# norlab-ulaval/mask_bev

Hardware: AMD Instinct MI355X
Metric: LiDAR scans/sec fwd+bwd, 120k-pt 512x512 BEV 100q (higher is better)
Workload: dtype bf16; 1 GPU; semantic_kitti_512: 120000 pts/scan, 512x512 BEV, 100 queries; scans_per_gpu=4, global_batch=4, parallelism=dp1, step=fwd + Hungarian loss + bwd + AdamW; inputs device-resident, launch=hip-graph, tuned_gemm_table=True, k3_adam_fused=True

## Files before the change

include/maskbev_hip.h:

```cpp
#ifndef MASKBEV_HIP_H_
#define MASKBEV_HIP_H_

#include <stddef.h>
#include <stdint.h>

#ifdef __cplusplus
extern "C" {
#endif

typedef enum {
  MBV_OK = 0,
  MBV_ERR_BAD_ARG = -1,
  MBV_ERR_WORKSPACE = -2,
  MBV_ERR_UNSUPPORTED = -3
} mbv_status;

int mbv_abi_version(void);

#define MBV_DT_F32 0
#define MBV_DT_BF16 1
#define MBV_DT_F16 2

size_t mbv_voxelize_workspace_bytes(int64_t total_points, int32_t batch, int64_t cells_per_scan);

// ... 377 lines not shown
int mbv_groupnorm_fwd(const void* x, int32_t x_dtype, int64_t batch, int32_t channels, int32_t h, int32_t w,
                      int32_t groups, const float* gamma, const float* beta, float eps, const void* add,
                      int32_t add_dtype, int32_t add_h, int32_t add_w, int32_t relu, void* y, int32_t y_dtype, float* mean,
                      float* rstd, void* workspace, size_t workspace_bytes, void* stream);
int mbv_groupnorm_bwd(const void* dy, int32_t dy_dtype, const void* x, int32_t x_dtype, const float* mean,
                      const float* rstd, const float* gamma, const float* beta, int64_t batch, int32_t channels, int32_t h,
                      int32_t w, int32_t groups, int32_t relu, void* dx, int32_t dx_dtype, float* dgamma, float* dbeta,
                      int32_t accumulate, float* plane_sums, void* stream);

size_t mbv_gemm16_tn_group_workspace_bytes(const int64_t* m, const int64_t* n, const int64_t* k, int32_t count);

int mbv_gemm16_tn_group(const void* const* g, const void* const* x, float* const* dw, const int64_t* m, const int64_t* n,
                        const int64_t* k, const int64_t* ldg, const int64_t* ldx, int32_t count, int32_t dtype,
                        void* workspace, size_t workspace_bytes, void* stream);

#define MBV_RC_LOAD 0
#define MBV_RC_STORE 1
#define MBV_RC_GEMM 2
#define MBV_RC_LN 3
#define MBV_RC_LN_BWD 4
#define MBV_RC_ADD 5
#define MBV_RC_COLSUM 6
#define MBV_RC_FFN 7
#define MBV_RC_FFN_IO 8
#define MBV_RC_SUM 9
#define MBV_RC_ACCUM 4
#define MBV_RC_RELU 8
#define MBV_RC_MASK 16
#define MBV_RC_SAVE_SUM 32
#define MBV_RC_SLICE 64
#define MBV_RC_SPLIT 64
#define MBV_RC_FRAG 128
#define MBV_RC_OWNER(j) (((j) + 1) << 8)
#define MBV_TR_MAX 96
typedef struct MbvRowStage {
  int32_t op;
  int16_t dst, src, src2, reserved;
  int32_t n, k, flags, ld, ld2;
  const void* p0;
  const void* p1;
  const void* p2;
} MbvRowStage;
int mbv_rowchain_max_stages(void);
int mbv_rowchain_slots(void);
int mbv_rowchain_run(const MbvRowStage* stages, int32_t num_stages, int32_t rows, int32_t q_mod, float eps,
                     int32_t wdtype, void* stream);
int mbv_rowchain_run_split(const MbvRowStage* stages, int32_t num_stages, int32_t rows, int32_t q_mod, float eps,
                           int32_t wdtype, int32_t split, void* stream);
int mbv_fragment_group(const void* const* src, void* const* dst, const int32_t* rows, const int32_t* cols,
                       const int32_t* ld, const int32_t* transposed, int32_t n, void* stream);
int mbv_copy_group(const void* const* src, void* const* dst, const int64_t* bytes, int32_t n, void* stream);
int mbv_transpose_group(const void* const* src, void* const* dst, const int32_t* rows, const int32_t* cols, int32_t n,
                        int32_t elem_size, void* stream);

int mbv_gemm32s_supported(int32_t layout, int64_t m, int64_t n, int64_t k);

int mbv_f32_absmax_group(const float* const* x, const int64_t* rows, const int64_t* cols, const int64_t* ld,
                         uint32_t* const* out, int32_t count, void* stream);

int mbv_ln_bound_group(const float* const* gamma, const float* const* beta, const int32_t* c, uint32_t* const* records,
                       int32_t count, void* stream);

int mbv_gemm32s_nt(const float* x, const float* w, const float* bias, float* out, float* out_pre, int64_t m, int64_t n,
                   int64_t k, int64_t ldx, int64_t ldw, int64_t ldo, const uint32_t* amax_x, const uint32_t* amax_w,
                   uint32_t* amax_out, int32_t act, int32_t batch, int64_t stride_x, int64_t stride_w, int64_t stride_o,
                   void* stream);

int mbv_gemm32s_nn(const float* g, const float* w, float* out, int64_t m, int64_t n, int64_t k, int64_t ldg, int64_t ldw,
                   int64_t ldo, const uint32_t* amax_g, const uint32_t* amax_w, uint32_t* amax_out, int32_t batch,
                   int64_t stride_g, int64_t stride_w, int64_t stride_o, void* stream);

size_t mbv_gemm32s_tn_workspace_bytes(int64_t m, int64_t n, int64_t k);
int mbv_gemm32s_tn_acc(const float* g, const float* x, float* dw, int64_t m, int64_t n, int64_t k, int64_t ldg, int64_t ldx,
                       const uint32_t* amax_g, const uint32_t* amax_x, void* workspace, size_t workspace_bytes,
                       void* stream);

int mbv_patch_embed32_supported(int64_t batch, int64_t channels, int64_t h, int64_t w, int64_t embed);
int mbv_patch_embed32_fwd(const float* image, const float* weight, const float* bias, float* out, int64_t batch,
                          int64_t channels, int64_t h, int64_t w, int64_t embed, const uint32_t* amax_image,
                          const uint32_t* amax_w, void* stream);
int mbv_patch_embed32_bwd_image(const float* d_out, const float* weight, float* d_image, int64_t batch, int64_t channels,
                                int64_t h, int64_t w, int64_t embed, const uint32_t* amax_g, const uint32_t* amax_w,
                                void* stream);
size_t mbv_patch_embed32_bwd_weight_workspace_bytes(int64_t batch, int64_t channels, int64_t h, int64_t w, int64_t embed);
int mbv_patch_embed32_bwd_weight(const float* d_out, const float* image, float* d_weight, int64_t batch, int64_t channels,
                                 int64_t h, int64_t w, int64_t embed, const uint32_t* amax_g, const uint32_t* amax_image,
                                 void* workspace, size_t workspace_bytes, void* stream);


size_t mbv_gemm32s_tn_group_workspace_bytes(const int64_t* m, const int64_t* n, const int64_t* k, int32_t count);
int mbv_gemm32s_tn_group(const float* const* g, const float* const* x, float* const* dw, const int64_t* m, const int64_t* n,
                         const int64_t* k, const int64_t* ldg, const int64_t* ldx, const uint32_t* const* amax_g,
                         const uint32_t* const* amax_x, int32_t count, void* workspace, size_t workspace_bytes, void* stream);

int64_t mbv_conv_rows(int64_t batch, int64_t H, int64_t W);
int mbv_conv_pad_rows(const void* src, void* dst, int64_t batch, int64_t C, int64_t H, int64_t W, int32_t elem_size, void* stream);
int mbv_conv_unpad_rows(const void* src, void* dst, int64_t batch, int64_t C, int64_t H, int64_t W, int32_t elem_size,
                        void* stream);
int mbv_conv3x3_gemm32s(const float* rows, const float* wm, float* out_rows, int64_t batch, int64_t H, int64_t W, int64_t C,
                        int64_t cout, const uint32_t* amax_rows, const uint32_t* amax_w, uint32_t* amax_out, void* stream);
int mbv_conv3x3_gemm16(const void* rows, const void* wm, void* out_rows, int64_t batch, int64_t H, int64_t W, int64_t C,
                       int64_t cout, int32_t dtype, int32_t out_f32, void* stream);

int64_t mbv_gemm32s_nn_part_rows(int64_t m, int32_t batch);
int mbv_gemm32s_nn_act(const float* g, const float* w, float* out, const float* pre, float* parts, size_t parts_bytes,
                       int64_t m, int64_t n, int64_t k, int64_t ldg, int64_t ldw, int64_t ldo, int64_t ldpre,
// ... 25 lines not shown
```

mask_bev_amd/_lib.py:

```python
from __future__ import annotations

import ctypes
import os
from ctypes import c_double, c_float, c_int32, c_int64, c_size_t, c_void_p
from typing import Dict, List, Tuple

_PKG_DIR = os.path.dirname(os.path.abspath(__file__))
LIB_PATH = os.path.join(_PKG_DIR, 'libmaskbev_hip.so')

ABI_VERSION = 59


class MaskBevHipError(RuntimeError):
    pass


_P = c_void_p
_F = c_float
_I = c_int32
_L = c_int64
_D = c_double

SIGNATURES: Dict[str, Tuple[object, List[object]]] = {
    'mbv_abi_version': (ctypes.c_int, []),
    'mbv_voxelize_workspace_bytes': (c_size_t, [_L, _I, _L]),
    'mbv_voxelize': (ctypes.c_int, [_P, _I, _L, _P, _I, _F, _F, _F, _F, _F, _F, _F, _F, _F, _I, _I, _I, _I, _I, _I, _L,
                                    _P, _P, _P, _P, _P, _P, _P, c_size_t, _P]),
    'mbv_gather_voxels': (ctypes.c_int, [_P, _I, _P, _L, _I, _P, _P]),
    'mbv_pfn_decorate': (ctypes.c_int, [_P, _I, _P, _P, _P, _P, _L, _I, _F, _F, _F, _F, _F, _F, _P, _P, _P]),
    'mbv_pfn_stats': (ctypes.c_int, [_P, _P, _P, _P, _P, _L, _I, _I, _P, _P]),
    'mbv_pfn_bn_finalize': (ctypes.c_int, [_P, c_double, _P, _P, _F, _F, _I, _P, _P, _I, _P, _P, _P, _P, _P]),
    'mbv_pfn_apply_max': (ctypes.c_int, [_P, _P, _P, _P, _P, _P, _L, _I, _I, _P, _P, _P, _P]),
    'mbv_pfn_bwd_route': (ctypes.c_int, [_P, _P, _P, _P, _P, _P, _P, _I, _P, _P, _P, _P, _L, _I, _I, _P, _P, _P]),
    'mbv_pfn_bwd_bn': (ctypes.c_int, [_P, _P, _P, _P, _P, _P, _P, _P, c_double, _I, _P, _P, _L, _I, _I, _P, _P]),
    'mbv_scatter_layernorm_workspace_bytes': (c_size_t, [_I]),
    'mbv_scatter_layernorm_patch_supported': (ctypes.c_int, [_I, _I, _I, _I]),
    'mbv_scatter_layernorm_fwd': (ctypes.c_int, [_P, _P, _P, _P, _P, _I, _I, _I, _I, _F, _I, _I, _P, _P, _P, c_size_t,
                                                 _P, _P, _P]),
    'mbv_scatter_layernorm_fwd2': (ctypes.c_int, [_P, _P, _P, _P, _P, _I, _I, _I, _I, _F, _I, _I, _P, _P, _P, c_size_t,
                                                  _P, _P, _P, _P]),
    'mbv_scatter_layernorm_bwd': (ctypes.c_int, [_P, _I, _I, _P, _P, _P, _P, _P, _I, _I, _I, _I, _L, _P, _P, _P, _I, _P,
                                                 c_size_t, _P, _P, _P]),
    'mbv_scatter_layernorm_bwd_adamw': (ctypes.c_int, [_P, _I, _I, _P, _P, _P, _P, _P, _P, _I, _I, _I, _I, _L, _P, _P, _P, _P, _P,
                                                       _P, _P, _I, _F, _F, _F, _F, _F, _L, _I, _P, c_size_t, _P, _P, _P]),
    'mbv_msda_prepare_supported': (ctypes.c_int, [_I, _I]),
    'mbv_pfn_forward_layout': (ctypes.c_int64, [_L, _L, _P, _I, _P]),
    'mbv_pfn_forward': (ctypes.c_int, [_P, _I, _P, _P, _P, _L, _L, _I, _P, _P, _P, _P, _P, _P, _I, _F, _F, _I, _P, _L, _P]),
    'mbv_skinny_gemm_f32_addrows': (ctypes.c_int, [_P, _P, _P, _L, _I, _I, _I, _P, _P, _P]),
    'mbv_skinny_gemm_f32_supported': (ctypes.c_int, [_L, _I, _I]),
    'mbv_skinny_gemm_f32': (ctypes.c_int, [_P, _P, _P, _L, _I, _I, _I, _I, _P]),
    'mbv_msda_prepare_fwd': (ctypes.c_int, [_P, _P, _I, _P, _P, _I, _I, _I, _I, _I, _P, _P, _P]),
    'mbv_msda_prepare_fwd_ld': (ctypes.c_int, [_P, _L, _P, _L, _P, _P, _I, _P, _P, _I, _I, _I, _I, _I, _P, _P, _P]),
    'mbv_msda_prepare_bwd': (ctypes.c_int, [_P, _P, _P, _P, _I, _I, _I, _I, _I, _I, _P, _P, _P]),
    'mbv_msda_prepare_bwd_ld': (ctypes.c_int, [_P, _P, _P, _P, _I, _I, _I, _I, _I, _I, _P, _L, _P, _L, _P]),
    'mbv_ms_deform_attn_fwd': (ctypes.c_int, [_P, _P, _P, _P, _P, _I, _I, _I, _I, _I, _I, _I, _P, _P]),
    'mbv_ms_deform_attn_fwd_v': (ctypes.c_int, [_P, _I, _P, _P, _P, _P, _I, _I, _I, _I, _I, _I, _I, _P, _P]),
    'mbv_ms_deform_attn_bwd_locattn': (ctypes.c_int, [_P, _P, _I, _P, _P, _P, _P, _I, _I, _I, _I, _I, _I, _I, _P, _P, _P]),
    'mbv_ms_deform_attn_bwd_split': (ctypes.c_int, [_I, _I, _P]),
    'mbv_ms_deform_attn_bwd_value_packed_supported': (ctypes.c_int, [_I, _I, _I, _I, _P]),
    'mbv_ms_deform_attn_bwd_value_packed_workspace_bytes': (c_size_t, [_I, _I, _I, _I]),
    'mbv_ms_deform_attn_bwd_value_packed': (ctypes.c_int, [_P, _P, _P, _I, _I, _I, _I, _I, _I, _I, _P, _P, _I, _L, _P, c_size_t, _P]),
    'mbv_ms_deform_attn_bwd': (ctypes.c_int, [_P, _P, _P, _P, _P, _P, _I, _I, _I, _I, _I, _I, _I, _P, _P, _P, _P, _I,
                                              _P]),
    'mbv_rowchain_max_stages': (ctypes.c_int, []),
    'mbv_rowchain_slots': (ctypes.c_int, []),
    'mbv_rowchain_run': (ctypes.c_int, [_P, _I, _I, _I, _F, _I, _P]),
    'mbv_rowchain_run_split': (ctypes.c_int, [_P, _I, _I, _I, _F, _I, _I, _P]),
    'mbv_transpose_group': (ctypes.c_int, [_P, _P, _P, _P, _I, _I, _P]),
    'mbv_copy_group': (ctypes.c_int, [_P, _P, _P, _I, _P]),
    'mbv_fragment_group': (ctypes.c_int, [_P, _P, _P, _P, _P, _P, _I, _P]),
    'mbv_window_attn_lse_elems': (_L, [_I, _I, _I, _I, _I]),
    'mbv_window_attn_fwd': (ctypes.c_int, [_P, _P, _P, _I, _I, _I, _I, _I, _I, _I, _I, _P, _P, _P]),
    'mbv_window_attn_bwd': (ctypes.c_int, [_P, _P, _P, _P, _P, _P, _I, _I, _I, _I, _I, _I, _I, _I, _P, _P, _P, _I, _I, _P]),
    'mbv_point_sample_fwd': (ctypes.c_int, [_P, _P, _P, _P, _I, _I, _I, _I, _P, _P]),
    'mbv_point_sample_bwd': (ctypes.c_int, [_P, _P, _P, _P, _I, _I, _I, _I, _L, _P, _P]),
    'mbv_point_sample_bwd_stack': (ctypes.c_int, [_P, _P, _P, _P, _I, _I, _I, _I, _I, _I, _I, _P, _I, _P]),
    'mbv_hungarian': (ctypes.c_int, [_P, _I, _I, _I, _P, _P]),
    'mbv_hungarian_padded': (ctypes.c_int, [_P, _I, _I, _I, _P, _P, _P]),
    'mbv_hungarian_wide_t': (ctypes.c_int, [_P, _I, _I, _I, _P, _P]),
    'mbv_select_uncertain_points': (ctypes.c_int, [_P, _P, _L, _I, _I, _P, _P]),
    'mbv_adamw_step': (ctypes.c_int, [_P, _P, _P, _P, _P, _I, _L, _F, _F, _F, _F, _F, _L, _F, _I, _I, _P, _P, _P, _P]),
    'mbv_grad_nonfinite': (ctypes.c_int, [_P, _L, _P, _P]),
    'mbv_loss_scale_update': (ctypes.c_int, [_P, _P, _P, _F, _F, _I, _P, _P]),
    'mbv_refresh_shadow': (ctypes.c_int, [_P, _P, _I, _L, _P]),
    'mbv_colsum_accum': (ctypes.c_int, [_P, _I, _L, _I, _P, _P]),
    'mbv_act_bwd_colsum': (ctypes.c_int, [_P, _P, _I, _I, _L, _I, _P, _P, _P]),
    'mbv_wgrad_small_f32': (ctypes.c_int, [_P, _P, _I, _I, _I, _P, _P, _P]),
    'mbv_wgrad_small_f32_group': (ctypes.c_int, [_P, _P, _P, _P, _P, _P, _P, _I, _P]),
    'mbv_mask_loss_rows_fwd': (ctypes.c_int, [_P, _P, _L, _I, _P, _P]),
    'mbv_mask_loss_rows_bwd': (ctypes.c_int, [_P, _P, _P, _L, _I, _P, _P]),
    'mbv_dice_bce_reduce': (ctypes.c_int, [_P, _L, _I, _F, _F, _P, _P, _P, _P]),
    'mbv_mask_loss_rows_bwd_coef': (ctypes.c_int, [_P, _P, _P, _P, _I, _P, _I, _L, _I, _I, _P, _P]),
    'mbv_sample_select_uncertain': (ctypes.c_int, [_P, _P, _P, _P, _L, _I, _I, _I, _I, _P, _I, _P, _P]),
    'mbv_uniform_points': (ctypes.c_int, [_P, _L, _I, _P, _P]),
    'mbv_add_layernorm_supported': (ctypes.c_int, [_I]),
    'mbv_add_layernorm_bwd_blocks': (_L, [_L, _I]),
    'mbv_add_layernorm_fwd': (ctypes.c_int, [_P, _I, _P, _I, _P, _P, _L, _I, _F, _P, _P, _I, _P, _P, _P]),
    'mbv_add_layernorm_fwd2': (ctypes.c_int, [_P, _I, _P, _I, _L, _P, _P, _L, _I, _F, _P, _P, _I, _P, _I, _P, _P, _P]),
    'mbv_transposed_batch_sum_accum': (ctypes.c_int, [_P, _I, _L, _I, _P, _P]),
    'mbv_add_layernorm_bwd': (ctypes.c_int, [_P, _I, _P, _I, _P, _P, _P, _P, _L, _I, _P, _P, _I, _P, _P, _I, _P, _P,
                                             _I, _P]),
    'mbv_add_layernorm_bwd2': (ctypes.c_int, [_P, _I, _P, _I, _P, _I, _P, _P, _P, _P, _L, _I, _P, _P, _I, _P, _P, _I, _P,
                                              _P, _I, _P]),
    'mbv_add_layernorm_bwd3': (ctypes.c_int, [_P, _I, _P, _I, _P, _I, _P, _P, _P, _P, _L, _I, _P, _P, _I, _P, _P, _I, _P,
                                              _P, _I, _P, _P]),
    'mbv_add_layernorm_bwd_direct': (ctypes.c_int, [_L, _I]),
    'mbv_merge_layernorm_supported': (ctypes.c_int, [_I, _I, _I]),
    'mbv_merge_layernorm_fwd': (ctypes.c_int, [_P, _L, _I, _I, _I, _P, _P, _F, _P, _I, _P, _P, _P]),
    'mbv_merge_layernorm_bwd': (ctypes.c_int, [_P, _I, _P, _P, _P, _P, _L, _I, _I, _I, _P, _P, _P, _I, _P, _I, _P]),
    'mbv_colsum_accum_group': (ctypes.c_int, [_P, _P, _P, _P, _P, _P, _I, _P]),
    'mbv_instance_ids': (ctypes.c_int, [_P, _I, _I, _I, _I, _I, _P, _P, _P, _P]),
    'mbv_expand_instance_masks': (ctypes.c_int, [_P, _P, _I, _I, _I, _I, _P, _P, _P]),
    'mbv_matched_mask_iou': (ctypes.c_int, [_P, _P, _P, _P, _I, _I, _I, _I, _I, _P, _P, _P]),
    'mbv_match_cost_terms': (ctypes.c_int, [_P, _L, _I, _I, _I, _P, _P, _P]),
    'mbv_match_cost': (ctypes.c_int, [_P, _P, _P, _P, _L, _I, _I, _I, _I, _I, _P, _P]),
    'mbv_match_products_supported': (ctypes.c_int, [_I, _I, _I]),
    'mbv_match_products': (ctypes.c_int, [_P, _P, _L, _I, _I, _I, _I, _P, _P, _P]),
    'mbv_match_cost_split': (ctypes.c_int, [_P, _P, _P, _P, _L, _I, _I, _I, _I, _I, _I, _P, _P]),
    'mbv_cls_loss_fwd': (ctypes.c_int, [_P, _P, _P, _P, _I, _I, _I, _I, _I, _F, _F, _P, _P, _P]),
    'mbv_cls_loss_bwd': (ctypes.c_int, [_P, _P, _P, _P, _P, _P, _I, _I, _I, _I, _I, _F, _F, _P, _P]),
    'mbv_packed_mask_words': (_L, [_I, _I]),
    'mbv_pack_binary_masks': (ctypes.c_int, [_P, _L, _I, _I, _P, _P]),
# ... 118 lines not shown
```

mask_bev_amd/mask2former_head.py:

```python
from __future__ import annotations

import contextlib
from typing import Dict, List, Optional, Sequence, Tuple

import numpy as np
import torch
import torch.nn as nn

from . import ops, switches
from .layers import ConvGN, FFN, conv1x1, LayerNorm, Linear, MultiScaleDeformableAttention, MultiheadAttention, sine_positional_encoding


class _DeformEncoderLayer(nn.Module):
    def __init__(self, embed_dims, num_heads, num_levels, num_points, ffn_channels):
        super().__init__()
        self.self_attn = MultiScaleDeformableAttention(embed_dims, num_heads, num_levels, num_points)
        self.ffn = FFN(embed_dims, ffn_channels, act='relu')
        self.norms = nn.ModuleList([LayerNorm(embed_dims), LayerNorm(embed_dims)])

    def forward(self, q, pos, ref, shapes, shapes_t, level_start, q_branch=None, fanout=False, pos_share=None,
                pos_share_index=0, wcat=None):
        c = q.shape[-1]
        ob, fb = self.self_attn.output_proj.bias, self.ffn.layers[1].bias
        d1, d2 = ops.bias_grad_deferrable(ob, c), ops.bias_grad_deferrable(fb, c)
# ... 314 lines not shown
        self.importance_sample_ratio = train_cfg.get('importance_sample_ratio', 0.75)
        self.class_weight = list(loss_cls.get('class_weight', [1.0] * self.num_classes + [0.1]))
        self.loss_cls_weight = float(loss_cls.get('loss_weight', 2.0))
        self.loss_mask_weight = float((loss_mask or {}).get('loss_weight', 5.0))
        self.loss_dice_weight = float((loss_dice or {}).get('loss_weight', 5.0))
        self.point_seed: Optional[int] = None
        self._iota_cache: Dict = {}
        self._side_streams: Dict = {}
        self.binary_gt_masks = True
        self.world_size_fn = None

    def init_weights(self):
        self.pixel_decoder.init_weights()
        for p in self.transformer_decoder.parameters():
            if p.dim() > 1:
                nn.init.xavier_normal_(p)

    def _forward_head(self, decoder_out, mask_feature, target_size, out=None):
        x = self.transformer_decoder.post_norm(decoder_out)
        cls_pred = self.cls_embed(x)
        mask_embed = self.mask_embed(x)
        mask_pred, blocked = ops.mask_logits(mask_embed, mask_feature, target_size, out)
        return cls_pred, mask_pred, blocked

    @staticmethod
    def _target_key(t):
        if isinstance(t, ops.PackedMasks):
            t = t.words
        if not torch.is_tensor(t) or not t.is_cuda:
            return None
        return (t.data_ptr(), tuple(t.shape), t.dtype)

    def announce_targets(self, gt_labels, gt_masks) -> None:
        keys = (self._target_key(gt_labels), self._target_key(gt_masks))
        self._announced_targets = keys if None not in keys else None

    def forward(self, x: List[torch.Tensor], batch_data_samples=None):
        bs = x[0].shape[0]
        self._early_event = None
        announced, self._announced_targets = getattr(self, '_announced_targets', None), None
        if (announced is not None and x[0].is_cuda and self.training and torch.is_grad_enabled()
                and switches.get('early_targets')):
            self._early_event = (torch.cuda.Event(), announced)
            self._early_event[0].record(torch.cuda.current_stream(x[0].device))
        mask_features, memories = self.pixel_decoder(x)
        dec_in, dec_pos, dec_key = [], [], []
        adt = (torch.get_autocast_dtype('cuda') if (torch.is_autocast_enabled('cuda') and memories[0].is_cuda)
               else memories[0].dtype)
        for i in range(self.num_transformer_feat_level):
            m = memories[i]
            h, w = m.shape[-2:]
            dec_pos.append(sine_positional_encoding(h, w, self.decoder_embed_dims // 2, m.device)
                           .flatten(2).transpose(1, 2))
            a, k = ops.level_inputs(m, self.level_embed.weight, i, dec_pos[-1], adt)
            dec_in.append(a)
            dec_key.append(k)
        query_feat = self.query_feat.weight.unsqueeze(0).expand(bs, -1, -1)
        query_embed = self.query_embed.weight.unsqueeze(0).expand(bs, -1, -1)
        cls_list, mask_list = [], []
        nd = len(self.transformer_decoder.layers) + 1
        stack = torch.empty((nd, bs, self.num_queries) + tuple(mask_features.shape[-2:]), dtype=torch.float32,
                            device=mask_features.device) if mask_features.is_cuda else None
        self._mask_stack = stack
        self._stack_sink = None
        self._gq_stash = None
        deferred = (stack is not None and self.training and torch.is_grad_enabled()
                    and switches.get('deferred_heads'))
        if deferred:
            self._stack_sink = ops.StackGradSink(nd, bs, self.num_queries, mask_features.dtype, mask_features.device)
        feats_q = [query_feat]

        def heads(qf, size, slot):
            if not deferred:
                return self._forward_head(qf, mask_features, size, slot)
            with torch.no_grad():
                return self._forward_head(qf, mask_features, size, slot)

        cls_pred, mask_pred, blocked = heads(query_feat, memories[0].shape[-2:], None if stack is None else stack[0])
        cls_list.append(cls_pred)
        mask_list.append(mask_pred)
        nl = self.num_transformer_feat_level
        layers = self.transformer_decoder.layers
        shared = [None] * len(layers)
        if (ops.shared_kv_supported(self.num_queries, mask_features.device)
                and switches.get('shared_kv')):
            for lvl in range(nl):
                idx = [i for i in range(len(layers)) if i % nl == lvl]
                holder, token = ops.shared_kv_project(
                    dec_key[lvl], dec_in[lvl],
                    [(layers[i].cross_attn.attn.in_proj_weight, layers[i].cross_attn.attn.in_proj_bias) for i in idx])
                for slot, i in enumerate(idx):
                    shared[i] = (holder, token, slot)
        if self._fused_decoder_ok(mask_features, shared, deferred):
            return self._forward_decoder_fused(query_feat, query_embed, mask_features, memories, shared, stack, deferred,
                                               cls_list, mask_list, blocked, feats_q)
        query_branch = None
        for i, layer in enumerate(layers):
            lvl = i % nl
            if i + 1 < len(layers):
                query_feat, query_branch = layer(query_feat, dec_in[lvl], query_embed, dec_pos[lvl], blocked,
                                                 dec_key[lvl], shared[i], query_branch=query_branch, fanout=True)
            else:
                query_feat = layer(query_feat, dec_in[lvl], query_embed, dec_pos[lvl], blocked, dec_key[lvl], shared[i],
                                   query_branch=query_branch)
                query_branch = query_feat
            feats_q.append(query_branch)
            cls_pred, mask_pred, blocked = heads(query_branch, memories[(i + 1) % nl].shape[-2:],
# ... 306 lines not shown
```

mask_bev_amd/ops_attention.py:

```python
from __future__ import annotations

import ctypes
from dataclasses import dataclass
from typing import List, Optional, Sequence

import torch

from . import _lib, switches
from ._lib import MaskBevHipError, check
from .ops_core import *
from .ops_records import *
from .ops_gemm import *


class _WindowAttention(torch.autograd.Function):
    @staticmethod
    def forward(ctx, qkv, qkv_bias, bias_table, num_heads, ws, shift, full_bias_grad=False):
        lib = _lib.load()
        _need_gpu(qkv, qkv_bias, bias_table)
        ctx.full_bias_grad = full_bias_grad
        if qkv.dtype not in _ACT_DTYPES:
            raise MaskBevHipError(f'window_attention supports f32, bf16 and fp16 qkv, got {qkv.dtype}')
        qkv = qkv.contiguous()
        b, h, w, c3 = qkv.shape
# ... 207 lines not shown
        t = key_in.numel() // e
        dk2, dv2 = dk.view(t, n * e), dv.view(t, n * e)
        key2, val2 = key_in.reshape(t, e), val_in.reshape(t, e).to(dk.dtype)
        f32 = dk2.dtype == torch.float32 and dk2.is_cuda
        if ctx.needs_input_grad[1]:
            grads[1] = (mm32_nn(dk2, wk) if f32 else dk2.mm(wk)).view_as(key_in)
        if ctx.needs_input_grad[2]:
            grads[2] = (mm32_nn(dv2, wv) if f32 else dv2.mm(wv)).view_as(val_in).to(val_in.dtype)
        def _arena(p):
            return getattr(p, '_mbv_arena', False) and p.grad is not None and p.grad.dtype == torch.float32
        if all(_arena(ctx.params[i]) and ctx.needs_input_grad[3 + i] for i in range(2 * n)):
            for j in range(n):
                w, b_ = ctx.params[2 * j], ctx.params[2 * j + 1]
                for g2, x2, r0 in ((dk2, key2, e), (dv2, val2, 2 * e)):
                    _wgrad_into(w.grad[r0:r0 + e], g2[:, j * e:(j + 1) * e], x2, None, persistent=True)
                    if not _defer_colsum(g2, b_.grad[r0:r0 + e], t, e, n * e, offset=j * e):
                        _colsum_now(g2, b_.grad[r0:r0 + e], t, e, n * e, offset=j * e)
                _fire_grad_hooks(w)
                _fire_grad_hooks(b_)
            return tuple(grads)
        gw = torch.zeros((2, n * e, e), dtype=torch.float32, device=dk.device)
        gb = torch.zeros((2, n * e), dtype=torch.float32, device=dk.device)
        _wgrad_into(gw[0], dk2, key2)
        _wgrad_into(gw[1], dv2, val2)
        colsum_accum(dk2, gb[0])
        colsum_accum(dv2, gb[1])
        dst, src = [], []
        for j in range(n):
            w, b_ = ctx.params[2 * j], ctx.params[2 * j + 1]
            rows = slice(j * e, (j + 1) * e)
            for p, g, slot in ((w, gw, 3 + 2 * j), (b_, gb, 4 + 2 * j)):
                if not ctx.needs_input_grad[slot]:
                    continue
                if getattr(p, '_mbv_arena', False) and p.grad is not None and p.grad.dtype == torch.float32:
                    dst += [p.grad[e:2 * e], p.grad[2 * e:3 * e]]
                    src += [g[0][rows], g[1][rows]]
                else:
                    full = torch.zeros_like(p)
                    full[e:2 * e] = g[0][rows]
                    full[2 * e:3 * e] = g[1][rows]
                    grads[slot] = full
        if dst:
            torch._foreach_add_(dst, src)
            for j in range(n):
                _fire_grad_hooks(ctx.params[2 * j])
                _fire_grad_hooks(ctx.params[2 * j + 1])
        return tuple(grads)


class _LevelInputs(torch.autograd.Function):

    @staticmethod
    def forward(ctx, memory, level_weight, index, pos, dtype):
        b, c = memory.shape[:2]
        x = memory.flatten(2).transpose(1, 2) + level_weight[index].view(1, 1, -1)
        key = x + pos
        ctx.index, ctx.mem_shape, ctx.mem_dtype = index, memory.shape, memory.dtype
        ctx.level_weight = level_weight
        return x.to(dtype), key.to(dtype)

    @staticmethod
    def backward(ctx, g_in, g_key):
        w, i = ctx.level_weight, ctx.index
        b, c = ctx.mem_shape[:2]
        if g_in is None and g_key is None:
            return None, None, None, None, None
        if g_in is None or g_key is None:
            g = (g_in if g_key is None else g_key).float()
        else:
            g = torch.add(g_in.float(), g_key)
        g_mem = g.transpose(1, 2).reshape(ctx.mem_shape).to(ctx.mem_dtype) if ctx.needs_input_grad[0] else None
        g_w = None
        if ctx.needs_input_grad[1]:
            g2 = g.reshape(-1, c)
            if getattr(w, '_mbv_arena', False) and w.grad is not None and w.grad.dtype == torch.float32 and g2.is_cuda:
                colsum_accum(g2, w.grad[i], persistent=True)
                _fire_grad_hooks(w)
            else:
                g_w = torch.zeros_like(w)
                g_w[i] = g2.sum(0).to(w.dtype)
        return g_mem, g_w, None, None, None


class _LevelPositions(torch.autograd.Function):

    @staticmethod
    def forward(ctx, weight, lengths, *pos):
        ctx.lengths = lengths
        ctx.weight = weight
        out = torch.cat([p + weight[i].view(1, 1, -1) for i, p in enumerate(pos)], 1)
        return out

    @staticmethod
    def backward(ctx, g):
        w, lengths = ctx.weight, ctx.lengths
        c = g.shape[-1]
        g2 = g.reshape(-1, c) if g.shape[0] == 1 else g.sum(0)
        g2 = g2.contiguous()
        direct = (getattr(w, '_mbv_arena', False) and w.grad is not None and w.grad.dtype == torch.float32
                  and w.grad.is_contiguous() and g2.is_cuda and g2.dtype in _ACT_DTYPES)
        gw = None if direct else torch.zeros_like(w)
        start = 0
        for i, n in enumerate(lengths):
            if direct:
                if not _defer_colsum(g2, w.grad[i], n, c, c, offset=start * c):
                    _colsum_now(g2, w.grad[i], n, c, c, offset=start * c)
            else:
                gw[i] = g2[start:start + n].sum(0).to(w.dtype)
            start += n
        if direct:
            _fire_grad_hooks(w)
        return (gw, None) + (None,) * len(lengths)


def level_positions(weight: torch.Tensor, pos) -> torch.Tensor:
    return _LevelPositions.apply(weight, tuple(int(p.shape[1]) for p in pos), *pos)


def level_inputs(memory: torch.Tensor, level_weight: torch.Tensor, index: int, pos: torch.Tensor, dtype: torch.dtype):
    return _LevelInputs.apply(memory, level_weight, index, pos, dtype)


def shared_kv_project(key_in: torch.Tensor, val_in: torch.Tensor, packed_params) -> tuple:
    holder = SharedKV()
    flat = [t for wb in packed_params for t in wb]
    token = _SharedKVProject.apply(holder, key_in, val_in, *flat)
    return holder, token


def shared_kv_supported(num_queries: int, device) -> bool:
    return device.type == 'cuda' and num_queries <= 128


class _AttentionSharedKV(torch.autograd.Function):
    @staticmethod
    def forward(ctx, q, token, blocked, num_heads, holder, slot):
        lib = _lib.load()
        k_cat, v_cat = holder.k_cat, holder.v_cat
        _need_gpu(q, k_cat, v_cat, blocked)
        dt = k_cat.dtype
        if dt not in _ACT_DTYPES:
            raise MaskBevHipError(f'attention supports f32, bf16 and fp16, got {dt}')
        ctx.q_dtype = q.dtype
        q = q.to(dt).contiguous()
        b, nq, e = q.shape
        nl = k_cat.shape[1]
        d = e // num_heads
        ld = holder.n * e
        off = slot * e * k_cat.element_size()
        mask = None
        if blocked is not None:
            mask = blocked.reshape(b, nq, nl).contiguous()
            mask = mask.view(torch.uint8) if mask.dtype == torch.bool else mask.to(torch.uint8)
        out = torch.empty_like(q)
        lse = torch.empty((b, num_heads, nq), dtype=torch.float32, device=q.device)
        ws = _workspace(lib.mbv_attn_workspace_bytes(b, nq, nl, num_heads, d), q.device)
        kp, vp = ctypes.c_void_p(k_cat.data_ptr() + off), ctypes.c_void_p(v_cat.data_ptr() + off)
        if _k6_split(dt, num_heads, d, ld, q, out) and (k_cat.data_ptr() + off) % 16 == 0 and (v_cat.data_ptr() + off) % 16 == 0:
            check(lib.mbv_attn_split_fwd_ld(_ptr(q), kp, vp, ld, _ptr(mask), b, nq, nl, num_heads, d, _ptr(out), _ptr(lse),
                                            _ptr(ws), ws.numel(), _stream()), 'mbv_attn_split_fwd_ld')
        else:
            rc = lib.mbv_attn_fwd_ld(_ptr(q), kp, vp, ld, _ptr(mask), _dt_flag(dt), b, nq, nl, num_heads, d, _ptr(out),
                                     _ptr(lse), _ptr(ws), ws.numel(), _stream())
            check(rc, 'mbv_attn_fwd_ld')
        ctx.save_for_backward(q, mask, out, lse)
        ctx.holder, ctx.slot, ctx.num_heads = holder, slot, num_heads
        return out

    @staticmethod
    def backward(ctx, grad_out):
        lib = _lib.load()
        q, mask, out, lse = ctx.saved_tensors
        holder, slot, h = ctx.holder, ctx.slot, ctx.num_heads
# ... 118 lines not shown
```

Before: 180.4 scans/s.

## Fuse per-level input/key token construction into one grouped transpose-add kernel

Adds a HIP kernel that, for all decoder feature levels in a single launch, transposes channel-major memory to token-major, adds the level embedding and positional encoding, and writes the value and key tensors in the activation dtype. A matching backward kernel sums the value and key gradients, transposes them back to the memory layout and emits the f32 per-token sums used for the level-embedding gradient. Level positions also go through the same forward kernel. This replaces several separate elementwise, transpose and cast ops per level with one launch each direction, at the cost of extra validation code and a materialised f32 gradient buffer for the embedding column sums.

```diff
diff --git a/include/maskbev_hip.h b/include/maskbev_hip.h
--- a/include/maskbev_hip.h
+++ b/include/maskbev_hip.h
@@ -453,6 +453,13 @@
 int mbv_copy_group(const void* const* src, void* const* dst, const int64_t* bytes, int32_t n, void* stream);
 int mbv_transpose_group(const void* const* src, void* const* dst, const int32_t* rows, const int32_t* cols, int32_t n,
                         int32_t elem_size, void* stream);
+int mbv_level_tokens_fwd(const void* const* src, int32_t src_dtype, const void* const* row, const void* const* pos,
+                         const int64_t* pos_strides, const int32_t* lengths, int32_t n_levels, int32_t batch,
+                         int32_t channels, void* const* out_val, void* const* out_key, const int64_t* out_batch_stride,
+                         int32_t out_dtype, void* stream);
+int mbv_level_tokens_bwd(const void* const* g_val, const void* const* g_key, int32_t g_dtype, const int32_t* lengths,
+                         int32_t n_levels, int32_t batch, int32_t channels, void* const* g_sum, void* const* g_src,
+                         int32_t src_dtype, void* stream);
 
 int mbv_gemm32s_supported(int32_t layout, int64_t m, int64_t n, int64_t k);
 
diff --git a/mask_bev_amd/_lib.py b/mask_bev_amd/_lib.py
--- a/mask_bev_amd/_lib.py
+++ b/mask_bev_amd/_lib.py
@@ -68,6 +68,8 @@
     'mbv_rowchain_run_split': (ctypes.c_int, [_P, _I, _I, _I, _F, _I, _I, _P]),
     'mbv_transpose_group': (ctypes.c_int, [_P, _P, _P, _P, _I, _I, _P]),
     'mbv_copy_group': (ctypes.c_int, [_P, _P, _P, _I, _P]),
+    'mbv_level_tokens_fwd': (ctypes.c_int, [_P, _I, _P, _P, _P, _P, _I, _I, _I, _P, _P, _P, _I, _P]),
+    'mbv_level_tokens_bwd': (ctypes.c_int, [_P, _P, _I, _P, _I, _I, _I, _P, _P, _I, _P]),
     'mbv_fragment_group': (ctypes.c_int, [_P, _P, _P, _P, _P, _P, _I, _P]),
     'mbv_window_attn_lse_elems': (_L, [_I, _I, _I, _I, _I]),
     'mbv_window_attn_fwd': (ctypes.c_int, [_P, _P, _P, _I, _I, _I, _I, _I, _I, _I, _I, _P, _P, _P]),
diff --git a/mask_bev_amd/csrc/level_tokens.hip b/mask_bev_amd/csrc/level_tokens.hip
--- /dev/null
+++ b/mask_bev_amd/csrc/level_tokens.hip
@@ -0,0 +1,220 @@
+#include "common.hpp"
+
+namespace {
+constexpr int LT_MAX = 8;
+constexpr int LT_TC = 64;
+constexpr int LT_TL = 32;
+
+struct LtLevel {
+  const void* a;
+  const void* b;
+  const float* row;
+  void* o0;
+  void* o1;
+  long pos_bs, pos_ls, pos_cs;
+  long o0_bs, o1_bs;
+  int L, tiles_l, tile_begin;
+};
+struct LtArgs {
+  int n, B, C, tiles_c;
+  int dt_cm;
+  int dt_tm;
+  LtLevel e[LT_MAX];
+};
+
+__device__ __forceinline__ float lt_load(const void* p, long i, int dt) {
+  if (dt == MBV_DT_F32) return reinterpret_cast<const float*>(p)[i];
+  const unsigned short h = reinterpret_cast<const unsigned short*>(p)[i];
+  if (dt == MBV_DT_BF16) return __uint_as_float((unsigned)h << 16);
+  return (float)__builtin_bit_cast(_Float16, h);
+}
+__device__ __forceinline__ unsigned short lt_bits(float f, int dt) {
+  if (dt == MBV_DT_BF16) return f32_to_bf16_rne(f);
+  return __builtin_bit_cast(unsigned short, (_Float16)f);
+}
+__device__ __forceinline__ void lt_store(void* p, long i, float f, int dt) {
+  if (dt == MBV_DT_F32) reinterpret_cast<float*>(p)[i] = f;
+  else reinterpret_cast<unsigned short*>(p)[i] = lt_bits(f, dt);
+}
+__device__ __forceinline__ void lt_load2(const void* p, long i, int dt, float& x, float& y) {
+  if (dt == MBV_DT_F32) {
+    const float2 v = *reinterpret_cast<const float2*>(reinterpret_cast<const float*>(p) + i);
+    x = v.x; y = v.y;
+  } else {
+    const unsigned v = *reinterpret_cast<const unsigned*>(reinterpret_cast<const unsigned short*>(p) + i);
+    if (dt == MBV_DT_BF16) { x = __uint_as_float(v << 16); y = __uint_as_float(v & 0xffff0000u); }
+    else { x = (float)__builtin_bit_cast(_Float16, (unsigned short)(v & 0xffffu)); y = (float)__builtin_bit_cast(_Float16, (unsigned short)(v >> 16)); }
+  }
+}
+__device__ __forceinline__ void lt_store2(void* p, long i, int dt, float x, float y) {
+  if (dt == MBV_DT_F32) *reinterpret_cast<float2*>(reinterpret_cast<float*>(p) + i) = make_float2(x, y);
+  else *reinterpret_cast<unsigned*>(reinterpret_cast<unsigned short*>(p) + i) = (unsigned)lt_bits(x, dt) | ((unsigned)lt_bits(y, dt) << 16);
+}
+
+struct LtTile { int level, b, c0, l0; };
+__device__ __forceinline__ LtTile lt_tile(const LtArgs& A) {
+  int ei = 0;
+  for (int i = 1; i < A.n; ++i)
+    if ((int)blockIdx.x >= A.e[i].tile_begin) ei = i;
+  const LtLevel& e = A.e[ei];
+  int t = (int)blockIdx.x - e.tile_begin;
+  const int per_b = A.tiles_c * e.tiles_l;
+  LtTile r;
+  r.level = ei;
+  r.b = t / per_b;
+  t -= r.b * per_b;
+  r.c0 = (t / e.tiles_l) * LT_TC;
+  r.l0 = (t % e.tiles_l) * LT_TL;
+  return r;
+}
+
+template <bool KEY>
+__global__ void __launch_bounds__(256) k_level_tokens_fwd(const LtArgs A) {
+  __shared__ float sv[LT_TC][LT_TL + 1];
+  __shared__ float sk[KEY ? LT_TC : 1][LT_TL + 1];
+  const LtTile T = lt_tile(A);
+  const LtLevel& e = A.e[T.level];
+  const int C = A.C, L = e.L;
+  {
+    const int tx = threadIdx.x & 31, ty = threadIdx.x >> 5;
+    const int l = T.l0 + tx;
+#pragma unroll
+    for (int k = 0; k < LT_TC / 8; ++k) {
+      const int cl = ty + 8 * k, c = T.c0 + cl;
+      if (l < L && c < C) {
+        const float x = lt_load(e.a, ((long)T.b * C + c) * L + l, A.dt_cm) + e.row[c];
+        sv[cl][tx] = x;
+        if (KEY) sk[cl][tx] = x + reinterpret_cast<const float*>(e.b)[T.b * e.pos_bs + l * e.pos_ls + c * e.pos_cs];
+      }
+    }
+  }
+  __syncthreads();
+  {
+    const int cl = (threadIdx.x & 31) * 2, ty = threadIdx.x >> 5;
+    const int c = T.c0 + cl;
+#pragma unroll
+    for (int k = 0; k < LT_TL / 8; ++k) {
+      const int ll = ty + 8 * k, l = T.l0 + ll;
+      if (l < L && c < C) {
+        lt_store2(e.o0, T.b * e.o0_bs + (long)l * C + c, A.dt_tm, sv[cl][ll], sv[cl + 1][ll]);
+        if (KEY) lt_store2(e.o1, T.b * e.o1_bs + (long)l * C + c, A.dt_tm, sk[cl][ll], sk[cl + 1][ll]);
+      }
+    }
+  }
+}
+
+__global__ void __launch_bounds__(256) k_level_tokens_bwd(const LtArgs A) {
+  __shared__ float sg[LT_TC][LT_TL + 1];
+  const LtTile T = lt_tile(A);
+  const LtLevel& e = A.e[T.level];
+  const int C = A.C, L = e.L;
+  {
+    const int cl = (threadIdx.x & 31) * 2, ty = threadIdx.x >> 5;
+    const int c = T.c0 + cl;
+#pragma unroll
+    for (int k = 0; k < LT_TL / 8; ++k) {
+      const int ll = ty + 8 * k, l = T.l0 + ll;
+      if (l < L && c < C) {
+        const long i = ((long)T.b * L + l) * C + c;
+        float x, y;
+        if (e.a && e.b) {
+          float u, v;
+          lt_load2(e.a, i, A.dt_tm, x, y);
+          lt_load2(e.b, i, A.dt_tm, u, v);
+          x += u; y += v;
+        } else {
+          lt_load2(e.a ? e.a : e.b, i, A.dt_tm, x, y);
+        }
+        if (e.o0) lt_store2(e.o0, i, MBV_DT_F32, x, y);
+        sg[cl][ll] = x;
+        sg[cl + 1][ll] = y;
+      }
+    }
+  }
+  __syncthreads();
+  {
+    const int tx = threadIdx.x & 31, ty = threadIdx.x >> 5;
+    const int l = T.l0 + tx;
+#pragma unroll
+    for (int k = 0; k < LT_TC / 8; ++k) {
+      const int cl = ty + 8 * k, c = T.c0 + cl;
+      if (l < L && c < C) lt_store(e.o1, ((long)T.b * C + c) * L + l, sg[cl][tx], A.dt_cm);
+    }
+  }
+}
+
+bool lt_dtype_ok(int dt) { return dt == MBV_DT_F32 || dt == MBV_DT_BF16 || dt == MBV_DT_F16; }
+bool lt_pair_aligned(const void* p, int dt) { return (reinterpret_cast<size_t>(p) & (dt == MBV_DT_F32 ? 7 : 3)) == 0; }
+
+long lt_plan(LtArgs& A, const int32_t* lengths, int n, int batch, int channels) {
+  A.n = n; A.B = batch; A.C = channels;
+  A.tiles_c = (channels + LT_TC - 1) / LT_TC;
+  long tiles = 0;
+  for (int i = 0; i < n; ++i) {
+    if (lengths[i] <= 0) return MBV_ERR_BAD_ARG;
+    A.e[i].L = lengths[i];
+    A.e[i].tiles_l = (lengths[i] + LT_TL - 1) / LT_TL;
+    A.e[i].tile_begin = (int)tiles;
+    tiles += (long)batch * A.tiles_c * A.e[i].tiles_l;
+    if (tiles > 0x7fffffffL) return MBV_ERR_UNSUPPORTED;
+  }
+  return tiles;
+}
+}
+
+extern "C" int mbv_level_tokens_fwd(const void* const* src, int32_t src_dtype, const void* const* row, const void* const* pos,
+                                    const int64_t* pos_strides, const int32_t* lengths, int32_t n_levels, int32_t batch,
+                                    int32_t channels, void* const* out_val, void* const* out_key, const int64_t* out_batch_stride,
+                                    int32_t out_dtype, void* stream_) {
+  hipStream_t stream = reinterpret_cast<hipStream_t>(stream_);
+  if (!src || !row || !lengths || !out_val || !out_batch_stride || n_levels <= 0 || batch <= 0 || channels <= 0)
+    return MBV_ERR_BAD_ARG;
+  if ((pos == nullptr) != (out_key == nullptr) || (pos && !pos_strides)) return MBV_ERR_BAD_ARG;
+  if (n_levels > LT_MAX || (channels & 1) || !lt_dtype_ok(src_dtype) || !lt_dtype_ok(out_dtype)) return MBV_ERR_UNSUPPORTED;
+  LtArgs A;
+  const long tiles = lt_plan(A, lengths, n_levels, batch, channels);
+  if (tiles < 0) return (int)tiles;
+  A.dt_cm = src_dtype; A.dt_tm = out_dtype;
+  for (int i = 0; i < n_levels; ++i) {
+    LtLevel& e = A.e[i];
+    if (!src[i] || !row[i] || !out_val[i] || (pos && (!pos[i] || !out_key[i]))) return MBV_ERR_BAD_ARG;
+    const int64_t bs = out_batch_stride[i];
+    if (bs < (int64_t)lengths[i] * channels || (bs & 1)) return MBV_ERR_BAD_ARG;
+    if (!lt_pair_aligned(out_val[i], out_dtype) || (pos && !lt_pair_aligned(out_key[i], out_dtype))) return MBV_ERR_BAD_ARG;
+    e.a = src[i]; e.row = reinterpret_cast<const float*>(row[i]);
+    e.b = pos ? pos[i] : nullptr;
+    e.o0 = out_val[i]; e.o1 = pos ? out_key[i] : nullptr;
+    e.pos_bs = pos ? pos_strides[3 * i] : 0; e.pos_ls = pos ? pos_strides[3 * i + 1] : 0; e.pos_cs = pos ? pos_strides[3 * i + 2] : 0;
+    if (e.pos_bs < 0 || e.pos_ls < 0 || e.pos_cs < 0) return MBV_ERR_BAD_ARG;
+    e.o0_bs = bs; e.o1_bs = (long)lengths[i] * channels;
+  }
+  if (pos) hipLaunchKernelGGL(k_level_tokens_fwd<true>, dim3((unsigned)tiles), dim3(256), 0, stream, A);
+  else hipLaunchKernelGGL(k_level_tokens_fwd<false>, dim3((unsigned)tiles), dim3(256), 0, stream, A);
+  MBV_CHECK_LAUNCH();
+  return MBV_OK;
+}
+
+extern "C" int mbv_level_tokens_bwd(const void* const* g_val, const void* const* g_key, int32_t g_dtype, const int32_t* lengths,
+                                    int32_t n_levels, int32_t batch, int32_t channels, void* const* g_sum, void* const* g_src,
+                                    int32_t src_dtype, void* stream_) {
+  hipStream_t stream = reinterpret_cast<hipStream_t>(stream_);
+  if (!g_val || !g_key || !lengths || !g_sum || !g_src || n_levels <= 0 || batch <= 0 || channels <= 0) return MBV_ERR_BAD_ARG;
+  if (n_levels > LT_MAX || (channels & 1) || !lt_dtype_ok(src_dtype) || !lt_dtype_ok(g_dtype)) return MBV_ERR_UNSUPPORTED;
+  LtArgs A;
+  const long tiles = lt_plan(A, lengths, n_levels, batch, channels);
+  if (tiles < 0) return (int)tiles;
+  A.dt_cm = src_dtype; A.dt_tm = g_dtype;
+  for (int i = 0; i < n_levels; ++i) {
+    LtLevel& e = A.e[i];
+    if ((!g_val[i] && !g_key[i]) || !g_src[i]) return MBV_ERR_BAD_ARG;
+    if ((g_val[i] && !lt_pair_aligned(g_val[i], g_dtype)) || (g_key[i] && !lt_pair_aligned(g_key[i], g_dtype)) ||
+        (g_sum[i] && !lt_pair_aligned(g_sum[i], MBV_DT_F32)))
+      return MBV_ERR_BAD_ARG;
+    e.a = g_val[i]; e.b = g_key[i]; e.row = nullptr;
+    e.o0 = g_sum[i]; e.o1 = g_src[i];
+    e.pos_bs = e.pos_ls = e.pos_cs = 0; e.o0_bs = e.o1_bs = 0;
+  }
+  hipLaunchKernelGGL(k_level_tokens_bwd, dim3((unsigned)tiles), dim3(256), 0, stream, A);
+  MBV_CHECK_LAUNCH();
+  return MBV_OK;
+}
diff --git a/mask_bev_amd/mask2former_head.py b/mask_bev_amd/mask2former_head.py
--- a/mask_bev_amd/mask2former_head.py
+++ b/mask_bev_amd/mask2former_head.py
@@ -390,7 +390,7 @@
             h, w = m.shape[-2:]
             dec_pos.append(sine_positional_encoding(h, w, self.decoder_embed_dims // 2, m.device)
                            .flatten(2).transpose(1, 2))
-            a, k = ops.level_inputs(m, self.level_embed.weight, i, dec_pos[-1], adt)
+        for a, k in ops.level_inputs_group(memories[:self.num_transformer_feat_level], self.level_embed.weight, dec_pos, adt):
             dec_in.append(a)
             dec_key.append(k)
         query_feat = self.query_feat.weight.unsqueeze(0).expand(bs, -1, -1)
diff --git a/mask_bev_amd/ops_attention.py b/mask_bev_amd/ops_attention.py
--- a/mask_bev_amd/ops_attention.py
+++ b/mask_bev_amd/ops_attention.py
@@ -283,7 +283,6 @@
 
     @staticmethod
     def forward(ctx, memory, level_weight, index, pos, dtype):
-        b, c = memory.shape[:2]
         x = memory.flatten(2).transpose(1, 2) + level_weight[index].view(1, 1, -1)
         key = x + pos
         ctx.index, ctx.mem_shape, ctx.mem_dtype = index, memory.shape, memory.dtype
@@ -293,7 +292,7 @@
     @staticmethod
     def backward(ctx, g_in, g_key):
         w, i = ctx.level_weight, ctx.index
-        b, c = ctx.mem_shape[:2]
+        c = ctx.mem_shape[1]
         if g_in is None and g_key is None:
             return None, None, None, None, None
         if g_in is None or g_key is None:
@@ -303,14 +302,96 @@
         g_mem = g.transpose(1, 2).reshape(ctx.mem_shape).to(ctx.mem_dtype) if ctx.needs_input_grad[0] else None
         g_w = None
         if ctx.needs_input_grad[1]:
-            g2 = g.reshape(-1, c)
-            if getattr(w, '_mbv_arena', False) and w.grad is not None and w.grad.dtype == torch.float32 and g2.is_cuda:
-                colsum_accum(g2, w.grad[i], persistent=True)
+            g_w = torch.zeros_like(w)
+            g_w[i] = g.reshape(-1, c).sum(0).to(w.dtype)
+        return g_mem, g_w, None, None, None
+
+
+def _f32_rows(weight: torch.Tensor, what: str) -> torch.Tensor:
+    w = weight.detach()
+    if w.dtype != torch.float32 or not w.is_contiguous() or w.dim() != 2:
+        raise MaskBevHipError(f'{what}: the level embedding must be a contiguous f32 (levels, C) matrix')
+    return w
+
+
+def _level_tokens_fwd(srcs, w, indices, pos, out_val, out_key, out_bs, what):
+    n = len(srcs)
+    b, c = int(srcs[0].shape[0]), int(srcs[0].shape[1])
+    if any(s.dtype != srcs[0].dtype or s.shape[:2] != srcs[0].shape[:2] or not s.is_contiguous() for s in srcs):
+        raise MaskBevHipError(f'{what}: the levels must share batch, channels and dtype')
+    P = ctypes.c_void_p * n
+    posp = strides = keyp = None
+    if pos is not None:
+        st = []
+        for p, s in zip(pos, srcs):
+            if p.dtype != torch.float32 or p.dim() != 3 or p.shape[0] not in (1, b) or p.shape[1] != s.shape[2] \
+                    or p.shape[2] != c:
+                raise MaskBevHipError(f'{what}: positions must be f32 (1 or B, L, C)')
+            st += [0 if p.shape[0] == 1 else p.stride(0), p.stride(1), p.stride(2)]
+        posp = P(*[p.data_ptr() for p in pos])
+        strides = (ctypes.c_int64 * (3 * n))(*st)
+        keyp = P(*[t.data_ptr() for t in out_key])
+    check(_lib.load().mbv_level_tokens_fwd(
+        P(*[s.data_ptr() for s in srcs]), _dt_flag(srcs[0].dtype), P(*[w.data_ptr() + 4 * c * int(i) for i in indices]),
+        posp, strides, (ctypes.c_int32 * n)(*[int(s.shape[2]) for s in srcs]), n, b, c,
+        P(*[t.data_ptr() for t in out_val]), keyp, (ctypes.c_int64 * n)(*out_bs), _dt_flag(out_val[0].dtype), _stream()),
+        'mbv_level_tokens_fwd')
+
+
+class _LevelInputsGroup(torch.autograd.Function):
+
+    @staticmethod
+    def forward(ctx, level_weight, indices, dtype, n, *mp):
+        memories, pos = mp[:n], mp[n:]
+        _need_gpu(level_weight, *memories, *pos)
+        w = _f32_rows(level_weight, 'level_inputs')
+        srcs = [m.detach().contiguous().flatten(2) for m in memories]
+        b, c = srcs[0].shape[:2]
+        if dtype not in _ACT_DTYPES:
+            raise MaskBevHipError(f'level_inputs: f32, bf16 or fp16 outputs, got {dtype}')
+        vals = [torch.empty((b, s.shape[2], c), dtype=dtype, device=s.device) for s in srcs]
+        keys = [torch.empty((b, s.shape[2], c), dtype=dtype, device=s.device) for s in srcs]
+        _level_tokens_fwd(srcs, w, indices, pos, vals, keys, [s.shape[2] * c for s in srcs], 'level_inputs')
+        ctx.level_weight, ctx.indices, ctx.n, ctx.dtype = level_weight, indices, n, dtype
+        ctx.mem_meta = [(m.shape, m.dtype) for m in memories]
+        ctx.set_materialize_grads(False)
+        return tuple(t for vk in zip(vals, keys) for t in vk)
+
+    @staticmethod
+    def backward(ctx, *g):
+        w, n, dt = ctx.level_weight, ctx.n, ctx.dtype
+        grads = [None] * (4 + 2 * n)
+        live = [i for i in range(n) if g[2 * i] is not None or g[2 * i + 1] is not None]
+        if not live:
+            return tuple(grads)
+        want_w = ctx.needs_input_grad[0]
+        b, c = ctx.mem_meta[0][0][:2]
+        dev = w.device
+        gv = [None if g[2 * i] is None else g[2 * i].to(dt).contiguous() for i in live]
+        gk = [None if g[2 * i + 1] is None else g[2 * i + 1].to(dt).contiguous() for i in live]
+        lens = [ctx.mem_meta[i][0][2] * ctx.mem_meta[i][0][3] for i in live]
+        g_sum = [torch.empty((b * l, c), dtype=torch.float32, device=dev) if want_w else None for l in lens]
+        g_mem = [torch.empty(ctx.mem_meta[i][0], dtype=ctx.mem_meta[i][1], device=dev) for i in live]
+        k = len(live)
+        P = ctypes.c_void_p * k
+        check(_lib.load().mbv_level_tokens_bwd(
+            P(*[None if t is None else t.data_ptr() for t in gv]), P(*[None if t is None else t.data_ptr() for t in gk]),
+            _dt_flag(dt), (ctypes.c_int32 * k)(*lens), k, b, c, P(*[None if t is None else t.data_ptr() for t in g_sum]),
+            P(*[t.data_ptr() for t in g_mem]), _dt_flag(g_mem[0].dtype), _stream()), 'mbv_level_tokens_bwd')
+        for j, i in enumerate(live):
+            if ctx.needs_input_grad[4 + i]:
+                grads[4 + i] = g_mem[j]
+        if want_w:
+            if getattr(w, '_mbv_arena', False) and w.grad is not None and w.grad.dtype == torch.float32:
+                for j, i in enumerate(live):
+                    colsum_accum(g_sum[j], w.grad[ctx.indices[i]], persistent=True)
                 _fire_grad_hooks(w)
             else:
                 g_w = torch.zeros_like(w)
-                g_w[i] = g2.sum(0).to(w.dtype)
-        return g_mem, g_w, None, None, None
+                for j, i in enumerate(live):
+                    g_w[ctx.indices[i]] += g_sum[j].sum(0).to(w.dtype)
+                grads[0] = g_w
+        return tuple(grads)
 
 
 class _LevelPositions(torch.autograd.Function):
@@ -319,7 +400,18 @@
     def forward(ctx, weight, lengths, *pos):
         ctx.lengths = lengths
         ctx.weight = weight
-        out = torch.cat([p + weight[i].view(1, 1, -1) for i, p in enumerate(pos)], 1)
+        if not weight.is_cuda:
+            return torch.cat([p + weight[i].view(1, 1, -1) for i, p in enumerate(pos)], 1)
+        _need_gpu(*pos)
+        w = _f32_rows(weight, 'level_positions')
+        c = int(w.shape[1])
+        if any(p.dim() != 3 or p.shape[0] != 1 or p.shape[2] != c or p.dtype != torch.float32 for p in pos):
+            raise MaskBevHipError('level_positions: f32 (1, N_i, C) encodings')
+        srcs = [p.detach().transpose(1, 2).contiguous() for p in pos]
+        out = torch.empty((1, sum(lengths), c), dtype=torch.float32, device=w.device)
+        starts = [sum(lengths[:i]) for i in range(len(lengths))]
+        _level_tokens_fwd(srcs, w, range(len(pos)), None, [out[0, s:] for s in starts], None,
+                          [sum(lengths) * c] * len(pos), 'level_positions')
         return out
 
     @staticmethod
@@ -348,8 +440,17 @@
     return _LevelPositions.apply(weight, tuple(int(p.shape[1]) for p in pos), *pos)
 
 
+def level_inputs_group(memories, level_weight: torch.Tensor, pos, dtype: torch.dtype, indices=None):
+    n = len(memories)
+    indices = tuple(range(n)) if indices is None else tuple(int(i) for i in indices)
+    if not memories[0].is_cuda:
+        return [_LevelInputs.apply(m, level_weight, i, p, dtype) for m, i, p in zip(memories, indices, pos)]
+    out = _LevelInputsGroup.apply(level_weight, indices, dtype, n, *memories, *pos)
+    return [(out[2 * i], out[2 * i + 1]) for i in range(n)]
+
+
 def level_inputs(memory: torch.Tensor, level_weight: torch.Tensor, index: int, pos: torch.Tensor, dtype: torch.dtype):
-    return _LevelInputs.apply(memory, level_weight, index, pos, dtype)
+    return level_inputs_group([memory], level_weight, [pos], dtype, indices=(index,))[0]
 
 
 def shared_kv_project(key_in: torch.Tensor, val_in: torch.Tensor, packed_params) -> tuple:
```

New measurement: 180.3 scans/s. Within noise of the previous version (-0.0%).
